# Azure/mmlspark

Hardware: NVIDIA H100
Metric: boosting_iters_per_sec (higher is better)
Workload: dtype int64 fixed-point histograms over u8 bins (fp32 gradients, fp64 split gains)

## Files before the change

mmlspark_b200/csrc/hist_kernel.cuh:

```cuda
#pragma once
#include <cstdint>
#include <cuda_runtime.h>
#include <cub/block/block_scan.cuh>

namespace b200gbm {

constexpr int kTileFeat = 32;
constexpr int kBins = 256;
constexpr int kLoBits = 18;
constexpr int kFlushRows = 1 << (32 - kLoBits);
#ifndef B200GBM_K4_EXPERIMENT
#define B200GBM_K4_EXPERIMENT 0
#endif
constexpr int kPlaneWords = kBins * kTileFeat;

struct HistWork {
  int begin;
  int count;
  int use_idx;
  int buf;
};

__global__ void __launch_bounds__(256)
k_gather_q(const HistWork* __restrict__ work, const int* __restrict__ idx0, const int* __restrict__ idx1, const int4* __restrict__ qgh,
           int4* __restrict__ qord) {
  const HistWork w = *work;
  if (!w.use_idx) return;
  const int* __restrict__ idx = w.buf ? idx1 : idx0;
  for (int i = blockIdx.x * blockDim.x + threadIdx.x; i < w.count; i += gridDim.x * blockDim.x) {
    const int p = w.begin + i;
    qord[p] = qgh[idx[p]];
  }
}

constexpr int kBoundBlockRows = 4096;
struct RowBlockBound {
  const int* prefix;
  int blocks;
};
inline int bound_blocks(int num_data) { return (num_data + kBoundBlockRows - 1) / kBoundBlockRows; }

__global__ void __launch_bounds__(256)
k_block_maxcnt(const uint8_t* __restrict__ bins, size_t rows_stride, int num_data, int num_columns, int* __restrict__ prefix) {
  __shared__ unsigned cnt[kBins * kTileFeat];
  __shared__ unsigned wmax[8];
  const int tile = blockIdx.y, tid = threadIdx.x;
  for (int e = tid; e < kBins * kTileFeat; e += blockDim.x) cnt[e] = 0u;
  __syncthreads();
  const int r0 = blockIdx.x * kBoundBlockRows, rows = min(kBoundBlockRows, num_data - r0);
  const unsigned* wp = reinterpret_cast<const unsigned*>(bins + (static_cast<size_t>(tile) * rows_stride + r0) * kTileFeat);
  for (int e = tid; e < rows * 8; e += blockDim.x) {
    const unsigned word = wp[e];
    const int c0 = (e & 7) * 4, rot = (e >> 3) & 3;
#pragma unroll
    for (int k = 0; k < 4; ++k) {
      const int kk = (k + rot) & 3;
      atomicAdd(&cnt[((word >> (8 * kk)) & 0xFFu) * kTileFeat + c0 + kk], 1u);
    }
  }
  __syncthreads();
  const int ncol = min(kTileFeat, num_columns - tile * kTileFeat);
  unsigned m = 0u;
  for (int e = tid; e < kBins * kTileFeat; e += blockDim.x)
    if ((e & (kTileFeat - 1)) < ncol) m = max(m, cnt[e]);
  m = __reduce_max_sync(0xffffffffu, m);
  if ((tid & 31) == 0) wmax[tid >> 5] = m;
  __syncthreads();
  if (tid == 0) {
    for (int i = 1; i < static_cast<int>(blockDim.x >> 5); ++i) m = max(m, wmax[i]);
    prefix[static_cast<size_t>(tile) * (gridDim.x + 1) + blockIdx.x] = static_cast<int>(m);
  }
}

__global__ void __launch_bounds__(1024) k_block_bound_prefix(int blocks, int* __restrict__ prefix) {
  using Scan = cub::BlockScan<int, 1024>;
  __shared__ typename Scan::TempStorage tmp;
  int* p = prefix + static_cast<size_t>(blockIdx.x) * (blocks + 1);
  int carry = 0;
  for (int b0 = 0; b0 < blocks; b0 += 1024) {
    const int b = b0 + threadIdx.x;
    const int v = b < blocks ? p[b] : 0;
    int ex, total;
    Scan(tmp).ExclusiveSum(v, ex, total);
    if (b < blocks) p[b] = carry + ex;
    carry += total;
    __syncthreads();
  }
  if (threadIdx.x == 0) p[blocks] = carry;
}

inline void launch_block_bound(const uint8_t* bins, size_t rows_stride, int num_data, int num_tiles, int num_columns, int* prefix,
                               cudaStream_t stream) {
  const int blocks = bound_blocks(num_data);
  if (blocks > 0) k_block_maxcnt<<<dim3(blocks, num_tiles), 256, 0, stream>>>(bins, rows_stride, num_data, num_columns, prefix);
  k_block_bound_prefix<<<num_tiles, 1024, 0, stream>>>(blocks, prefix);
}


__device__ __forceinline__ void cp_async16(void* smem, const void* gmem, bool valid) {
  unsigned s = static_cast<unsigned>(__cvta_generic_to_shared(smem));
  int sz = valid ? 16 : 0;
  asm volatile("cp.async.cg.shared.global [%0], [%1], 16, %2;\n" ::"r"(s), "l"(gmem), "r"(sz));
}
template <int N>
__device__ __forceinline__ void cp_async_wait() {
  asm volatile("cp.async.wait_group %0;\n" ::"n"(N));
}

constexpr int kWsConsumerWarps = 16;
constexpr int kWsProducerWarps = 2;
constexpr int kWsThreads = (kWsConsumerWarps + kWsProducerWarps) * 32;
constexpr int kWsStageRows = 512;
constexpr int kWsStages = 3;
constexpr int kFlushSlabBins = 32;
constexpr int kFlushRowBytes = kFlushSlabBins * 16;
constexpr int kFlushStageBytes = kTileFeat * kFlushRowBytes;
constexpr int kWsSmemBytes = 4 * kPlaneWords * 4 + kWsStages * (kWsStageRows * 32 + kWsStageRows * 16) + kFlushStageBytes + 64;
static_assert(kWsSmemBytes <= 227 * 1024, "K4 shared memory exceeds the 227 KB per block of sm_90");
static_assert(kFlushSlabBins * kTileFeat == 2 * kWsConsumerWarps * 32, "a flush slab is two (g,h) pairs per consumer thread");

__device__ __forceinline__ unsigned smem_u32(const void* p) { return static_cast<unsigned>(__cvta_generic_to_shared(p)); }
__device__ __forceinline__ void mbar_init(unsigned long long* bar, unsigned count) {
  asm volatile("mbarrier.init.shared::cta.b64 [%0], %1;\n" ::"r"(smem_u32(bar)), "r"(count));
}
__device__ __forceinline__ void mbar_arrive(unsigned long long* bar) {
  asm volatile("mbarrier.arrive.shared::cta.b64 _, [%0];\n" ::"r"(smem_u32(bar)) : "memory");
}
__device__ __forceinline__ void mbar_arrive_expect_tx(unsigned long long* bar, unsigned bytes) {
  asm volatile("mbarrier.arrive.expect_tx.shared::cta.b64 _, [%0], %1;\n" ::"r"(smem_u32(bar)), "r"(bytes) : "memory");
}
__device__ __forceinline__ void mbar_expect_tx(unsigned long long* bar, unsigned bytes) {
  asm volatile("mbarrier.expect_tx.relaxed.cta.shared::cta.b64 [%0], %1;\n" ::"r"(smem_u32(bar)), "r"(bytes) : "memory");
}
__device__ __forceinline__ void mbar_wait(unsigned long long* bar, unsigned parity) {
  asm volatile(
      "{\n"
      ".reg .pred p;\n"
      "WAIT_LOOP:\n"
      "mbarrier.try_wait.parity.shared::cta.b64 p, [%0], %1;\n"
      "@p bra DONE;\n"
      "bra WAIT_LOOP;\n"
      "DONE:\n"
      "}\n" ::"r"(smem_u32(bar)), "r"(parity) : "memory");
}
__device__ __forceinline__ void tma_bulk_g2s(void* smem_dst, const void* gmem_src, unsigned bytes, unsigned long long* bar) {
  asm volatile("cp.async.bulk.shared::cluster.global.mbarrier::complete_tx::bytes [%0], [%1], %2, [%3];\n" ::"r"(smem_u32(smem_dst)),
               "l"(gmem_src), "r"(bytes), "r"(smem_u32(bar))
               : "memory");
}
__device__ __forceinline__ void cp_async_mbar_arrive_noinc(unsigned long long* bar) {
  asm volatile("cp.async.mbarrier.arrive.noinc.shared::cta.b64 [%0];\n" ::"r"(smem_u32(bar)) : "memory");
}
__device__ __forceinline__ void bulk_reduce_add_u64(unsigned long long* gmem_dst, const void* smem_src, unsigned bytes) {
  asm volatile("cp.reduce.async.bulk.global.shared::cta.bulk_group.add.u64 [%0], [%1], %2;\n" ::"l"(gmem_dst), "r"(smem_u32(smem_src)),
               "r"(bytes)
               : "memory");
}
__device__ __forceinline__ void bulk_commit() { asm volatile("cp.async.bulk.commit_group;\n" ::: "memory"); }
__device__ __forceinline__ void bulk_wait_read_all() { asm volatile("cp.async.bulk.wait_group.read 0;\n" ::: "memory"); }
__device__ __forceinline__ void bulk_wait_all() { asm volatile("cp.async.bulk.wait_group 0;\n" ::: "memory"); }
__device__ __forceinline__ void fence_proxy_async_smem() { asm volatile("fence.proxy.async.shared::cta;\n" ::: "memory"); }

template <int NATOM>
__global__ void __launch_bounds__(kWsThreads, 1)
k4_hist_build_ws(const uint8_t* __restrict__ bins, size_t rows_stride, int num_tiles, const int4* __restrict__ qgh,
                 const int4* __restrict__ qord, const int* __restrict__ idx0, const int* __restrict__ idx1,
                 const HistWork* __restrict__ work, unsigned long long* __restrict__ hist, RowBlockBound bound) {
  extern __shared__ __align__(128) unsigned char smem_raw[];
  unsigned* plane = reinterpret_cast<unsigned*>(smem_raw);
  unsigned char* stage_bins = smem_raw + 4 * kPlaneWords * 4;
  int4* stage_q = reinterpret_cast<int4*>(stage_bins + kWsStages * kWsStageRows * 32);
  unsigned char* flush_stage = reinterpret_cast<unsigned char*>(stage_q) + kWsStages * kWsStageRows * 16;
  unsigned long long* full_bar = reinterpret_cast<unsigned long long*>(flush_stage + kFlushStageBytes);
  unsigned long long* empty_bar = full_bar + kWsStages;

  const HistWork w = *work;
  const int n = w.count;
  if (n <= 0) return;
  const int tid = threadIdx.x, lane = tid & 31, warp = tid >> 5;
  const int* __restrict__ idx = w.buf ? idx1 : idx0;

  long long cells_rows = static_cast<long long>(n) * num_tiles;
  int rpi = static_cast<int>((cells_rows + 4LL * gridDim.x - 1) / (4LL * gridDim.x));
  rpi = (rpi + kWsStageRows - 1) / kWsStageRows * kWsStageRows;
  rpi = max(rpi, kWsStageRows);
  rpi = min(rpi, kFlushRows);
  const int chunks = (n + rpi - 1) / rpi;
  const long long items = static_cast<long long>(chunks) * num_tiles;
  const int i0 = static_cast<int>(items * blockIdx.x / gridDim.x);
  const int i1 = static_cast<int>(items * (blockIdx.x + 1) / gridDim.x);
  if (i0 >= i1) return;

  if (tid == 0) {
    for (int i = 0; i < kWsStages; ++i) { mbar_init(&full_bar[i], kWsProducerWarps * 32); mbar_init(&empty_bar[i], kWsConsumerWarps); }
    asm volatile("fence.mbarrier_init.release.cluster;\n" ::: "memory");
  }
  for (int e = tid; e < 4 * kPlaneWords; e += kWsThreads) plane[e] = 0u;
  __syncthreads();

  unsigned gs = 0;
  if (warp >= kWsConsumerWarps) {
    const int ptid = tid - kWsConsumerWarps * 32;
    constexpr int kPT = kWsProducerWarps * 32;
    constexpr int kPerLane = kWsStageRows / kPT;
    for (int item = i0; item < i1; ++item) {
      const int tile = item / chunks, chunk = item - tile * chunks;
      const int row0 = chunk * rpi;
      const int nrows = min(rpi, n - row0);
      const int nst = (nrows + kWsStageRows - 1) / kWsStageRows;
      const uint8_t* tbins = bins + static_cast<size_t>(tile) * rows_stride * 32;
      for (int s = 0; s < nst; ++s, ++gs) {
        const int slot = gs % kWsStages;
        mbar_wait(&empty_bar[slot], ((gs / kWsStages) & 1u) ^ 1u);
        const int p0 = row0 + s * kWsStageRows;
        const int rows = min(kWsStageRows, row0 + nrows - p0);
        unsigned char* db = stage_bins + slot * kWsStageRows * 32;
        int4* dq = stage_q + slot * kWsStageRows;
        if (!w.use_idx) {
          if (ptid == 0) {
            mbar_arrive_expect_tx(&full_bar[slot], static_cast<unsigned>(rows) * 48u);
            const size_t r = static_cast<size_t>(w.begin + p0);
            tma_bulk_g2s(db, tbins + r * 32, static_cast<unsigned>(rows) * 32u, &full_bar[slot]);
            tma_bulk_g2s(dq, qgh + r, static_cast<unsigned>(rows) * 16u, &full_bar[slot]);
          } else {
            mbar_arrive(&full_bar[slot]);
          }
        } else {
          const int* ip = idx + w.begin + p0;
          if (ptid == 0) {
            mbar_expect_tx(&full_bar[slot], static_cast<unsigned>(rows) * 16u);
            tma_bulk_g2s(dq, qord + static_cast<size_t>(w.begin + p0), static_cast<unsigned>(rows) * 16u, &full_bar[slot]);
          }
          int rr[2 * kPerLane];
#pragma unroll
          for (int k = 0; k < 2 * kPerLane; ++k) { const int j = (ptid + k * kPT) >> 1; rr[k] = j < rows ? ip[j] : -1; }
#pragma unroll
          for (int k = 0; k < 2 * kPerLane; ++k) {
            const int hh = ptid + k * kPT, j = hh >> 1, half = (hh & 1) * 16;
            if (rr[k] >= 0) cp_async16(db + j * 32 + half, tbins + static_cast<size_t>(rr[k]) * 32 + half, true);
          }
          cp_async_mbar_arrive_noinc(&full_bar[slot]);
        }
      }
    }
    cp_async_wait<0>();
  } else {
#if B200GBM_K4_EXPERIMENT >= 1 && B200GBM_K4_EXPERIMENT <= 3
    unsigned exp_sink = 0;
#endif
    const int sub = lane >> 2, rot = lane & 3;
    auto item_rows = [&](int it, int& first, int& last) {
      const int t = it / chunks, r0 = (it - t * chunks) * rpi;
      first = w.begin + r0;
      last = first + min(rpi, n - r0) - 1;
      if (w.use_idx && bound.prefix) { first = idx[first]; last = idx[last]; }
    };
    auto item_bound = [&](int it, int first, int last) -> int {
      const int t = it / chunks, nr = min(rpi, n - (it - t * chunks) * rpi);
      if (!bound.prefix) return nr;
      const int* p = bound.prefix + static_cast<size_t>(t) * (bound.blocks + 1);
      return min(nr, p[last / kBoundBlockRows + 1] - p[first / kBoundBlockRows]);
    };
    int first, last;
    item_rows(i0, first, last);
    int next_bound = item_bound(i0, first, last);
    if (i0 + 1 < i1) item_rows(i0 + 1, first, last);
    int acc_bound = 0;
    for (int item = i0; item < i1; ++item) {
      const int tile = item / chunks, chunk = item - tile * chunks;
      const int row0 = chunk * rpi;
      const int nrows = min(rpi, n - row0);
      const int nst = (nrows + kWsStageRows - 1) / kWsStageRows;
      acc_bound += next_bound;
      next_bound = 0;
      if (item + 1 < i1) {
        next_bound = item_bound(item + 1, first, last);
        if (item + 2 < i1) item_rows(item + 2, first, last);
      }
      for (int s = 0; s < nst; ++s, ++gs) {
        const int slot = gs % kWsStages;
        mbar_wait(&full_bar[slot], (gs / kWsStages) & 1u);
        const int rows = min(kWsStageRows, nrows - s * kWsStageRows);
        const unsigned* sw = reinterpret_cast<const unsigned*>(stage_bins + slot * kWsStageRows * 32);
        const int4* sq = stage_q + slot * kWsStageRows;
        const int groups = (rows + 31) >> 5;
        for (int g = warp; g < groups; g += kWsConsumerWarps) {
          const int r = g * 32 + lane;
          if (r < rows) {
            const int4 q = sq[r];
            const unsigned* rw = sw + r * 8;
#pragma unroll
            for (int k = 0; k < 8; ++k) {
              const int w8 = (sub + k) & 7;
              const unsigned word = rw[w8];
#pragma unroll
              for (int j = 0; j < 4; ++j) {
                const int kk = (j + rot) & 3;
                const unsigned b = (word >> (8 * kk)) & 0xFFu;
                const unsigned a = b * 32u + static_cast<unsigned>(w8 * 4 + kk);
#if B200GBM_K4_EXPERIMENT == 0 || B200GBM_K4_EXPERIMENT == 4
                atomicAdd(&plane[a], static_cast<unsigned>(q.x));
                atomicAdd(&plane[kPlaneWords + a], static_cast<unsigned>(q.y));
                atomicAdd(&plane[2 * kPlaneWords + a], static_cast<unsigned>(q.z));
                if (NATOM == 4) atomicAdd(&plane[3 * kPlaneWords + a], static_cast<unsigned>(q.w));
#else
                if (B200GBM_K4_EXPERIMENT >= 2) atomicAdd(&plane[a], static_cast<unsigned>(q.x));
                if (B200GBM_K4_EXPERIMENT >= 3) atomicAdd(&plane[kPlaneWords + a], static_cast<unsigned>(q.y));
                if (B200GBM_K4_EXPERIMENT == 1) exp_sink ^= a + static_cast<unsigned>(q.x ^ q.y ^ q.z ^ q.w);
#endif
              }
            }
          }
        }
#if B200GBM_K4_EXPERIMENT >= 1 && B200GBM_K4_EXPERIMENT <= 3
        if (exp_sink == 0x12345679u) plane[lane] = exp_sink;
#endif
        __syncwarp();
        if (lane == 0) mbar_arrive(&empty_bar[slot]);
      }
      const bool flush = (item + 1 == i1) || ((item + 1) / chunks != tile) || (acc_bound + next_bound > kFlushRows);
      if (!flush) continue;
      acc_bound = 0;
      asm volatile("bar.sync 1, %0;\n" ::"n"(kWsConsumerWarps * 32) : "memory");
      unsigned long long* htile = hist + static_cast<size_t>(tile) * kTileFeat * kBins * 2;
      int sbin[2];
#pragma unroll
      for (int i = 0; i < 2; ++i) sbin[i] = (warp + i * kWsConsumerWarps + lane) & (kFlushSlabBins - 1);
      for (int b0 = 0; b0 < kBins; b0 += kFlushSlabBins) {
        long long g[2], h[2];
        bool nz = false;
#pragma unroll
        for (int i = 0; i < 2; ++i) {
          const int e = (b0 + sbin[i]) * kTileFeat + lane;
          const unsigned ghi = plane[e], glo = plane[kPlaneWords + e], hhi = plane[2 * kPlaneWords + e];
          const unsigned hlo = (NATOM == 4) ? plane[3 * kPlaneWords + e] : 0u;
          plane[e] = 0u;
          plane[kPlaneWords + e] = 0u;
          plane[2 * kPlaneWords + e] = 0u;
          if (NATOM == 4) plane[3 * kPlaneWords + e] = 0u;
          nz |= (ghi | glo | hhi | hlo) != 0u;
          g[i] = (static_cast<long long>(static_cast<int>(ghi)) << kLoBits) + static_cast<long long>(glo);
          h[i] = (NATOM == 4) ? (static_cast<long long>(static_cast<int>(hhi)) << kLoBits) + static_cast<long long>(hlo)
                              : static_cast<long long>(hhi);
        }
        if (tid == 0) bulk_wait_read_all();
        asm volatile("bar.sync 1, %0;\n" ::"n"(kWsConsumerWarps * 32) : "memory");
#pragma unroll
        for (int i = 0; i < 2; ++i)
          *reinterpret_cast<longlong2*>(flush_stage + lane * kFlushRowBytes + sbin[i] * 16) = make_longlong2(g[i], h[i]);
        fence_proxy_async_smem();
        int any;
        asm volatile(
            "{\n"
            ".reg .pred p, q;\n"
            "setp.ne.u32 p, %1, 0;\n"
            "bar.red.or.pred q, 1, %2, p;\n"
            "selp.s32 %0, 1, 0, q;\n"
            "}\n"
            : "=r"(any)
            : "r"(static_cast<unsigned>(nz)), "n"(kWsConsumerWarps * 32)
            : "memory");
#if B200GBM_K4_EXPERIMENT != 4
        if (tid == 0 && any) {
          for (int f = 0; f < kTileFeat; ++f)
            bulk_reduce_add_u64(htile + (static_cast<size_t>(f) * kBins + b0) * 2, flush_stage + f * kFlushRowBytes, kFlushSlabBins * 16);
          bulk_commit();
        }
#else
        (void)any; (void)htile;
#endif
      }
    }
    if (tid == 0) bulk_wait_all();
  }
}

inline cudaError_t set_k4_smem_limit() {
  const cudaError_t e = cudaFuncSetAttribute(k4_hist_build_ws<4>, cudaFuncAttributeMaxDynamicSharedMemorySize, kWsSmemBytes);
  if (e != cudaSuccess) return e;
  return cudaFuncSetAttribute(k4_hist_build_ws<3>, cudaFuncAttributeMaxDynamicSharedMemorySize, kWsSmemBytes);
}

inline void launch_k4(bool const_hessian, const uint8_t* bins, size_t rows_stride, int num_tiles, const int4* qgh, const int4* qord,
                      const int* idx0, const int* idx1, const HistWork* work, unsigned long long* hist, RowBlockBound bound, int grid,
                      cudaStream_t stream) {
  if (const_hessian)
    k4_hist_build_ws<3><<<grid, kWsThreads, kWsSmemBytes, stream>>>(bins, rows_stride, num_tiles, qgh, qord, idx0, idx1, work, hist, bound);
  else
    k4_hist_build_ws<4><<<grid, kWsThreads, kWsSmemBytes, stream>>>(bins, rows_stride, num_tiles, qgh, qord, idx0, idx1, work, hist, bound);
}

}
```

mmlspark_b200/csrc/tree_learner.cu:

```cuda
#include "tree_learner.h"

namespace b200gbm {

static size_t Align16(size_t x) { return (x + 15) & ~static_cast<size_t>(15); }
constexpr int kScanSmem = (768 + 64) * 8;
constexpr int kPartTickets = 8;

template <typename Fn>
static void ForEachTreeField(TreeDev& t, int L, Fn fn) {
  const size_t nodes = L - 1, leaves = L;
  fn(t.left_child, nodes); fn(t.right_child, nodes); fn(t.split_feature_inner, nodes); fn(t.threshold_bin, nodes);
  fn(t.decision_type, nodes); fn(t.split_gain, nodes); fn(t.leaf_value, leaves); fn(t.leaf_weight, leaves); fn(t.leaf_count, leaves);
  fn(t.internal_value, nodes); fn(t.internal_weight, nodes); fn(t.internal_count, nodes); fn(t.leaf_parent, leaves);
  fn(t.leaf_depth, leaves); fn(t.num_leaves, 1); fn(t.cat_bits, 8 * nodes); fn(t.cat_list, kCatListMax * nodes); fn(t.cat_list_len, nodes);
}
static size_t TreeBlobBytes(int L) {
  TreeDev t{};
  size_t bytes = 0;
  ForEachTreeField(t, L, [&](auto*& p, size_t count) { bytes += Align16(count * sizeof(*p)); });
  return bytes;
}
static TreeDev TreeBlobAt(unsigned char* base, int L) {
  TreeDev t{};
  size_t off = 0;
  ForEachTreeField(t, L, [&](auto*& p, size_t count) {
    p = reinterpret_cast<std::remove_reference_t<decltype(p)>>(base + off);
    off += Align16(count * sizeof(*p));
  });
  return t;
}

TreeLearner::TreeLearner(const Dataset& train, const Config& cfg, const Objective& obj, bool parallel, bool same_device, int num_sms,
                         cudaStream_t stream, Booster::Timing& timing)
    : train_(train), cfg_(cfg), parallel_(parallel), same_device_(same_device), num_sms_(num_sms), stream_(stream), timing_(timing) {
  const int n = train.num_data;
  const int L = cfg.num_leaves;
  cudaDeviceSetLimit(cudaLimitMaxL2FetchGranularity, 32);
  cudaGetLastError();
  B200_CUDA(set_k4_smem_limit());
  B200_CUDA(cudaFuncSetAttribute(k_scan, cudaFuncAttributeMaxDynamicSharedMemorySize, kScanSmem));

  ResetConfig(cfg);
  sp_.num_leaves = L; sp_.parallel = parallel_ ? 1 : 0;
  sp_.nf = train.nf; sp_.nf_pad = train.nf_pad; sp_.num_tiles = train.num_tiles; sp_.nfn = train.nfn;
  {
    sp_.cat_l2 = cfg.cat_l2; sp_.cat_smooth = cfg.cat_smooth;
    sp_.max_cat_threshold = cfg.max_cat_threshold; sp_.max_cat_to_onehot = cfg.max_cat_to_onehot;
    sp_.min_data_per_group = cfg.min_data_per_group; sp_.pad3 = 0;
    if (train.nw > 0) {
      if (sp_.max_cat_threshold > kCatListMax) Fatal("max_cat_threshold > " + std::to_string(kCatListMax) + " is not supported together with categorical features of more than 256 bins");
      if (sp_.max_cat_to_onehot > 256) Fatal("max_cat_to_onehot > 256 is not supported together with categorical features of more than 256 bins");
      B200_CUDA(cudaFuncSetAttribute(k4_hist_wide<4>, cudaFuncAttributeMaxDynamicSharedMemorySize, 4 * kWideHistSeg * 4));
      B200_CUDA(cudaFuncSetAttribute(k4_hist_wide<3>, cudaFuncAttributeMaxDynamicSharedMemorySize, 4 * kWideHistSeg * 4));
      B200_CUDA(cudaFuncSetAttribute(k_scan_wide, cudaFuncAttributeMaxDynamicSharedMemorySize, kWideMaxBins * 8));
    }
  }

  qgh_.Alloc(n); qord_.Alloc(n); idx0_.Alloc(n); idx1_.Alloc(n);
  slot_elems_ = train.hist_pairs * 2;
  H_.Alloc(slot_elems_); H_.Zero(stream_); pool_.Alloc(slot_elems_ * L);
  {
    int per_sm = 0;
    B200_CUDA(cudaOccupancyMaxActiveBlocksPerMultiprocessor(&per_sm, k_partition, 256, 0));
    int coop = 0;
    cudaDeviceGetAttribute(&coop, cudaDevAttrCooperativeLaunch, CurrentDevice());
    if (!coop || per_sm < 1) Fatal("this device cannot launch the cooperative partition kernel");
    part_max_blocks_ = per_sm * num_sms_;
  }
  flags_.Alloc(static_cast<size_t>(L) * train.nf_pad);
  cands_.Alloc(2 * static_cast<size_t>(train.nf_pad));
  leaves_.Alloc(L); ctrl_.Alloc(1); ctrl_.Zero(stream_);
  const int chunks = n / kPartChunk + 2;
  part_bits_.Alloc(static_cast<size_t>(chunks) * (kPartChunk / 32)); part_chunks_.Alloc(static_cast<size_t>(chunks) + chunks / kPartLocalScan + 8); part_chunks_.Zero(stream_);
  const size_t blob_bytes = TreeBlobBytes(L);
  tree_blob_.Alloc(blob_bytes);
  tree_dev_ = TreeAt(tree_blob_.p);
  B200_CUDA(cudaMemsetAsync(tree_blob_.p, 0, blob_bytes, stream_));
  B200_CUDA(cudaMallocHost(reinterpret_cast<void**>(&tree_host_), blob_bytes));
  B200_CUDA(cudaMallocHost(reinterpret_cast<void**>(&ctrl_host_), sizeof(TreeCtrl)));
  if (obj.RenewsLeaves()) {
    rn_keys_a_.Alloc(n); rn_keys_b_.Alloc(n); rn_pos_a_.Alloc(n); rn_pos_b_.Alloc(n); rn_leaf_of_pos_.Alloc(n); rn_leaf_a_.Alloc(n); rn_leaf_b_.Alloc(n);
    rn_res_.Alloc(n); rn_row_.Alloc(n); rn_seg_.Alloc(L + 1); rn_out_.Alloc(2 * static_cast<size_t>(L));
    if (obj.RenewWeights()) rn_cdf_.Alloc(n);
    size_t t1 = 0, t2 = 0;
    cub::DeviceRadixSort::SortPairs(nullptr, t1, rn_keys_a_.p, rn_keys_b_.p, rn_pos_a_.p, rn_pos_b_.p, n, 0, 64, stream_);
    cub::DeviceRadixSort::SortPairs(nullptr, t2, rn_leaf_a_.p, rn_leaf_b_.p, rn_pos_b_.p, rn_pos_a_.p, n, 0, 32, stream_);
    rn_tmp_bytes_ = std::max(t1, t2);
    rn_tmp_.Alloc(rn_tmp_bytes_ + 16);
  }
  col_rand_ = LcgRandom(cfg.feature_fraction_seed);
  feature_used_host_.assign(train.nf_pad, 0);
  for (int u = 0; u < train.nf; ++u) feature_used_host_[u] = 1;
  feature_used_.Alloc(train.nf_pad);
  feature_used_.Upload(feature_used_host_.data(), train.nf_pad, stream_);
  ResetFeaturesByTree();
}

TreeLearner::~TreeLearner() {
  if (split_op_trees_ > 0) {
    double tot = 0; for (auto& kv : split_op_ms_) tot += kv.second;
    fprintf(stderr, "[b200gbm split timing] %d trees, %.3f ms per tree in split operations:", split_op_trees_, tot / split_op_trees_);
    for (auto& kv : split_op_ms_) fprintf(stderr, " %s=%.1fus", kv.first.c_str(), 1000.0 * kv.second / split_op_trees_ / std::max(cfg_.num_leaves - 1, 1));
    fprintf(stderr, " (per split)\n");
  }
  if (tree_host_) cudaFreeHost(tree_host_);
  if (ctrl_host_) cudaFreeHost(ctrl_host_);
}

void TreeLearner::ResetConfig(const Config& cfg) {
  sp_.l1 = cfg.lambda_l1; sp_.l2 = cfg.lambda_l2; sp_.max_delta_step = cfg.max_delta_step; sp_.min_gain_to_split = cfg.min_gain_to_split;
  sp_.min_sum_hessian = cfg.min_sum_hessian_in_leaf; sp_.min_data_in_leaf = cfg.min_data_in_leaf; sp_.max_depth = cfg.max_depth;
}

TreeDev TreeLearner::TreeAt(unsigned char* blob) const { return TreeBlobAt(blob, sp_.num_leaves); }

void TreeLearner::ResetFeaturesByTree() {
  if (cfg_.feature_fraction >= 1.0) return;
  const int total = train_.nf;
  int cnt = std::max(static_cast<int>(total * cfg_.feature_fraction + 0.5), std::min(2, total));
  std::fill(feature_used_host_.begin(), feature_used_host_.end(), 0);
  for (int i : col_rand_.Sample(total, cnt)) feature_used_host_[train_.sample_order[i]] = 1;
  feature_used_.Upload(feature_used_host_.data(), train_.nf_pad, stream_);
}

void TreeLearner::Renew(const Objective& obj, const double* score_k, double rf_pred) {
  const int total = rows_;
  const int L = cfg_.num_leaves;
  cudaStream_t s = stream_;
  TreeCtrl* ctrl = ctrl_.p;
  const int egrid = num_sms_ * 8;
  const float* wptr = obj.RenewWeights();
  k_renew_gather<<<egrid, 256, 0, s>>>(ctrl, leaves_.p, idx0_.p, idx1_.p, train_.d_label.p, score_k, rf_pred,
                                       rn_keys_a_.p, rn_pos_a_.p, rn_res_.p, rn_leaf_of_pos_.p, rn_row_.p);
  size_t tb = rn_tmp_bytes_;
  B200_CUDA(cub::DeviceRadixSort::SortPairs(rn_tmp_.p, tb, rn_keys_a_.p, rn_keys_b_.p, rn_pos_a_.p, rn_pos_b_.p, total, 0, 64, s));
  k_renew_leaf_keys<<<egrid, 256, 0, s>>>(rn_pos_b_.p, rn_leaf_of_pos_.p, total, rn_leaf_a_.p);
  int leaf_bits = 1;
  while ((1 << leaf_bits) < L) ++leaf_bits;
  tb = rn_tmp_bytes_;
  B200_CUDA(cub::DeviceRadixSort::SortPairs(rn_tmp_.p, tb, rn_leaf_a_.p, rn_leaf_b_.p, rn_pos_b_.p, rn_pos_a_.p, total, 0, leaf_bits, s));
  k_renew_offsets<<<1, 32, 0, s>>>(ctrl, leaves_.p, rn_seg_.p);
  double* out = rn_out_.p;
  double* has = rn_out_.p + L;
  const int lgrid = (L + 127) / 128;
  if (!wptr) {
    k_renew_unweighted<<<lgrid, 128, 0, s>>>(ctrl, rn_seg_.p, rn_pos_a_.p, rn_res_.p, obj.RenewAlpha(), out, has);
  } else {
    k_renew_cdf<<<L, 1024, 0, s>>>(ctrl, rn_seg_.p, rn_pos_a_.p, rn_row_.p, wptr, rn_cdf_.p);
    k_renew_weighted<<<lgrid, 128, 0, s>>>(ctrl, rn_seg_.p, rn_pos_a_.p, rn_res_.p, rn_cdf_.p, obj.RenewAlpha(), out, has);
  }
  if (parallel_) Net().AllReduce(out, 2 * static_cast<size_t>(L), ncclDouble, ncclSum, s);
  k_renew_apply<<<lgrid, 128, 0, s>>>(ctrl, tree_dev_, out, has, parallel_ ? 1 : 0);
  B200_CUDA(cudaGetLastError());
  timing_.launches += wptr ? 7 : 6;
}

void TreeLearner::EnsureColumnCopy() {
  if (cols_tried_) return;
  cols_tried_ = true;
  const Dataset& d = train_;
  const char* env = std::getenv("B200GBM_COLUMN_COPY");
  if ((env && std::atoi(env) == 0) || d.nfn == 0) return;
  size_t free_b = 0, total_b = 0;
  const bool mem_ok = cudaMemGetInfo(&free_b, &total_b) == cudaSuccess;
  if (!mem_ok) cudaGetLastError();
  size_t share = 1;
  if (same_device_) {
    double arrived = 0.0;
    AllReduceHost(&arrived, 1, ncclSum, stream_);
    if (cudaMemGetInfo(&free_b, &total_b) != cudaSuccess) { cudaGetLastError(); free_b = 0; }
    double f = mem_ok ? static_cast<double>(free_b) : 0.0;
    AllReduceHost(&f, 1, ncclMin, stream_);
    free_b = static_cast<size_t>(f);
    share = static_cast<size_t>(Net().world);
  }
  if (!mem_ok || d.num_data == 0) return;
  const char* force = std::getenv("B200GBM_COLUMN_CACHE_COLUMNS");
  const size_t stride = (static_cast<size_t>(d.num_data) + 255) & ~static_cast<size_t>(255);
  const int ncols = d.num_tiles * 32;
  const size_t need = static_cast<size_t>(ncols) * stride;
  const size_t reserve = std::max<size_t>(static_cast<size_t>(8) << 30, total_b / 10);
  const size_t spare = free_b > reserve ? (free_b - reserve) / share : 0;
  const bool full = !force && spare >= need;
  int slots = ncols;
  if (!full) {
    slots = static_cast<int>(std::min<size_t>(d.num_columns, spare / stride));
    if (force) slots = std::min(slots, std::max(0, std::atoi(force)));
    if (slots == 0) return;
  }
  const size_t bytes = static_cast<size_t>(slots) * stride;
  uint8_t* p = nullptr;
  if (cudaMalloc(reinterpret_cast<void**>(&p), bytes) != cudaSuccess) { cudaGetLastError(); return; }
  bins_cols_.p = p; bins_cols_.n = bytes;
  cols_stride_ = stride;
  col_slot_host_.assign(ncols, -1);
  if (full) {
    for (int c = 0; c < ncols; ++c) col_slot_host_[c] = c;
    const long long work = ((static_cast<long long>(d.num_data) + 255) / 256) * d.num_tiles;
    k_tiles_to_columns<<<static_cast<unsigned>(std::min<long long>(work, static_cast<long long>(num_sms_) * 16)), 256, 0, stream_>>>(
        d.bins.p, d.rows_stride, d.num_tiles, d.num_data, bins_cols_.p, stride);
    B200_CUDA(cudaGetLastError());
  } else {
    slot_col_.assign(slots, -1);
    col_splits_.assign(ncols, 0);
  }
  col_slot_.Alloc(ncols);
  col_slot_.Upload(col_slot_host_.data(), ncols, stream_);
}

void TreeLearner::UpdateColumnCache(const HostTree& t) {
  if (slot_col_.empty()) return;
  const Dataset& d = train_;
  for (int i = 0; i + 1 < t.num_leaves; ++i) {
    const int f = t.split_feature_inner[i];
    if (f < d.nfn) ++col_splits_[d.meta_host[f].hist_off >> 8];
  }
  std::vector<int> cand;
  for (int c = 0; c < static_cast<int>(col_splits_.size()); ++c)
    if (col_splits_[c] > 0 && col_slot_host_[c] < 0) cand.push_back(c);
  std::stable_sort(cand.begin(), cand.end(), [&](int a, int b) { return col_splits_[a] > col_splits_[b]; });
  ColumnJobs jobs{};
  for (int c : cand) {
    if (jobs.n == kColumnBuildsMax) break;
    int slot = -1, victim = -1;
    for (int s = 0; s < static_cast<int>(slot_col_.size()) && slot < 0; ++s) {
      const int held = slot_col_[s];
      if (held < 0) slot = s;
      else if (victim < 0 || col_splits_[held] < col_splits_[slot_col_[victim]]) victim = s;
    }
    if (slot < 0) {
      if (col_splits_[slot_col_[victim]] >= col_splits_[c]) break;
      slot = victim;
      col_slot_host_[slot_col_[slot]] = -1;
      ++cache_evictions_;
    }
    slot_col_[slot] = c;
    col_slot_host_[c] = slot;
    jobs.col[jobs.n] = c; jobs.slot[jobs.n] = slot; ++jobs.n;
  }
  if (jobs.n == 0) return;
  const long long words = (static_cast<long long>(d.num_data) + 3) / 4;
  const unsigned gx = static_cast<unsigned>(std::max<long long>(1, std::min<long long>((words + 255) / 256, static_cast<long long>(num_sms_) * 8)));
  k_tiles_to_column_slots<<<dim3(gx, jobs.n), 256, 0, stream_>>>(d.bins.p, d.rows_stride, d.num_data, jobs, bins_cols_.p, cols_stride_);
  B200_CUDA(cudaGetLastError());
  col_slot_.Upload(col_slot_host_.data(), col_slot_host_.size(), stream_);
  cache_builds_ += jobs.n;
  timing_.launches += 1;
}

void TreeLearner::GetColumnCacheInfo(int64_t* out4) const {
  out4[0] = static_cast<int64_t>(slot_col_.size());
  out4[1] = static_cast<int64_t>(std::count_if(slot_col_.begin(), slot_col_.end(), [](int c) { return c >= 0; }));
  out4[2] = cache_builds_;
  out4[3] = cache_evictions_;
}

void TreeLearner::LaunchPartition(int grid, int last) {
  const Dataset& d = train_;
  TreeCtrl* ctrl = ctrl_.p;
  LeafState* leaves = leaves_.p;
  TreeDev tree = tree_dev_;
  uint8_t* flags = flags_.p;
  const FeatMeta* meta = d.meta.p;
  SplitParams sp = sp_;
  const uint8_t* bins = d.bins.p;
  size_t rows_stride = d.rows_stride;
  int* i0 = idx0_.p; int* i1 = idx1_.p;
  unsigned* bits = part_bits_.p;
  int* chunks = part_chunks_.p;
  const int4* qgh = qgh_.p;
  int4* qord = qord_.p;
  long long* H = H_.p;
  size_t h_elems = slot_elems_;
  const uint16_t* bins16 = d.bins16.p;
  int tickets_per_block = kPartTickets;
  const uint8_t* cols = bins_cols_.p;
  size_t cols_stride = cols_stride_;
  const int* col_slot = col_slot_.p;
  int* super_tot = part_chunks_.p + (d.num_data / kPartChunk + 2);
  const int* bundle_base = d.BundleBase();
  void* args[] = {&ctrl, &leaves, &tree, &flags, &meta, &sp, &last, &bins, &rows_stride, &i0, &i1, &bits, &chunks, &qgh, &qord, &H, &h_elems, &bins16, &tickets_per_block,
                  &cols, &cols_stride, &col_slot, &super_tot, &bundle_base};
  B200_CUDA(cudaLaunchCooperativeKernel(reinterpret_cast<void*>(k_partition), dim3(grid), dim3(256), args, 0, stream_));
}

void TreeLearner::Grow(const float* g, const float* h, bool const_hessian, const Bag* bag) {
  EnsureColumnCopy();
  const Dataset& d = train_;
  const int n = d.num_data;
  const int L = cfg_.num_leaves;
  rows_ = bag ? bag->count : n;
  TreeCtrl* ctrl = ctrl_.p;
  cudaStream_t s = stream_;
  const int egrid = num_sms_ * 8;
  nvtxRangePushA("b200gbm:K3 quantize + C1 root sums");
  B200_CUDA(cudaMemsetAsync(&ctrl->absmax_bits[0], 0, 8, s));
  k_absmax<<<egrid, 256, 0, s>>>(g, h, n, ctrl);
  if (parallel_) Net().AllReduce(&ctrl->absmax_bits[0], 2, ncclUint32, ncclMax, s);
  k_set_scale<<<1, 1, 0, s>>>(ctrl, const_hessian ? 1 : 0, 1.0);
  k_quantize<<<egrid, 256, 0, s>>>(g, h, n, qgh_.p, ctrl, const_hessian ? 1 : 0, bag ? bag->in_bag : nullptr, rows_);
  if (parallel_) Net().AllReduce(&ctrl->root_q[0], 3, ncclInt64, ncclSum, s);
  ResetFeaturesByTree();
  if (bag)
    B200_CUDA(cudaMemcpyAsync(idx0_.p, bag->rows, static_cast<size_t>(bag->count) * sizeof(int), cudaMemcpyDeviceToDevice, s));
  k_tree_init<<<1, 256, 0, s>>>(ctrl, leaves_.p, tree_dev_, flags_.p, sp_, rows_, feature_used_.p, bag ? 1 : 0);
  nvtxRangePop();
  timing_.launches += 4;
  const int pgrid = std::max(1, std::min(n / kPartChunk + 1, part_max_blocks_));
  const dim3 sgrid(std::max(1, d.nfn), 2);
  const RowBlockBound bound = d.BlockBound();
  static const bool split_timing = getenv("B200GBM_SPLIT_TIMING") != nullptr;
  auto mark = [&]() { if (split_timing) { cudaEvent_t e; cudaEventCreate(&e); cudaEventRecord(e, s); split_events_.push_back(e); } };
  k_round_ctl<<<1, 256, 0, s>>>(ctrl, leaves_.p, tree_dev_, flags_.p, d.meta.p, sp_, 0);
  timing_.launches += 1;
  for (int split = 0; split < L - 1; ++split) {
    mark();
    if (profile_hist) { cudaEvent_t a, b; B200_CUDA(cudaEventCreate(&a)); B200_CUDA(cudaEventCreate(&b)); hist_events_.push_back(a); hist_events_.push_back(b); B200_CUDA(cudaEventRecord(a, s)); }
    if (split == 0 && bag) k_gather_q<<<egrid, 256, 0, s>>>(&ctrl->hist_work, idx0_.p, idx1_.p, qgh_.p, qord_.p);
    mark();
    nvtxRangePushA("b200gbm:K4 histogram");
    launch_k4(const_hessian, d.bins.p, d.rows_stride, d.num_tiles, qgh_.p, qord_.p, idx0_.p, idx1_.p, &ctrl->hist_work,
              reinterpret_cast<unsigned long long*>(H_.p), bound, num_sms_, s);
    if (d.nw > 0) {
      int max_nb = 0;
      for (const WideMeta& wm : d.wide_host) max_nb = std::max(max_nb, wm.num_bin);
      const int segs = (max_nb + kWideHistSeg - 1) / kWideHistSeg;
      int units = 0;
      for (const WideMeta& wm : d.wide_host) units += (wm.num_bin + kWideHistSeg - 1) / kWideHistSeg;
      const dim3 wgrid(static_cast<unsigned>(std::max(1, std::min(64, 4 * num_sms_ / std::max(1, units)))), static_cast<unsigned>(d.nw), static_cast<unsigned>(segs));
      if (const_hessian)
        k4_hist_wide<3><<<wgrid, kWideThreads, 4 * kWideHistSeg * 4, s>>>(d.bins16.p, d.rows_stride, d.wide_meta.p, qgh_.p, qord_.p, idx0_.p, idx1_.p, &ctrl->hist_work,
                                                                         reinterpret_cast<unsigned long long*>(H_.p));
      else
        k4_hist_wide<4><<<wgrid, kWideThreads, 4 * kWideHistSeg * 4, s>>>(d.bins16.p, d.rows_stride, d.wide_meta.p, qgh_.p, qord_.p, idx0_.p, idx1_.p, &ctrl->hist_work,
                                                                         reinterpret_cast<unsigned long long*>(H_.p));
      timing_.launches += 1;
    }
    nvtxRangePop();
    if (profile_hist) B200_CUDA(cudaEventRecord(hist_events_.back(), s));
    mark();
    nvtxRangePushA(parallel_ ? "b200gbm:C2 histogram reduce + K5 scan + pick" : "b200gbm:K5 scan + pick");
    if (parallel_) Net().AllReduce(H_.p, slot_elems_, ncclInt64, ncclSum, s);
    mark();
    if (d.nw > 0) {
      k_scan_wide<<<dim3(d.nw, 2), 256, kWideMaxBins * 8, s>>>(ctrl, leaves_.p, d.wide_meta.p, H_.p, pool_.p, slot_elems_, flags_.p, cands_.p, sp_);
      timing_.launches += 1;
    }
    k_scan<<<sgrid, 256, (d.has_categorical || !d.bundles.empty()) ? kScanSmem : 0, s>>>(ctrl, leaves_.p, d.meta.p, H_.p, pool_.p, slot_elems_, flags_.p, cands_.p, sp_, d.BundleBase());
    nvtxRangePop();
    mark();
    nvtxRangePushA("b200gbm:K7 partition + controller");
    LaunchPartition(pgrid, split == L - 2 ? 1 : 0);
    nvtxRangePop();
    mark();
    timing_.launches += 3; timing_.hist_launches += 1;
  }
}

void TreeLearner::AddScore(double* score_k, double shrinkage) {
  k_add_score<<<num_sms_ * 8, 256, 0, stream_>>>(ctrl_.p, leaves_.p, tree_dev_, idx0_.p, idx1_.p, score_k, shrinkage);
}

void TreeLearner::ReadTree(HostTree* out) {
  const Dataset& d = train_;
  cudaStream_t s = stream_;
  B200_CUDA(cudaMemcpyAsync(tree_host_, tree_blob_.p, tree_blob_.n, cudaMemcpyDeviceToHost, s));
  B200_CUDA(cudaMemcpyAsync(ctrl_host_, ctrl_.p, sizeof(TreeCtrl), cudaMemcpyDeviceToHost, s));
  B200_CUDA(cudaStreamSynchronize(s));
  if (!split_events_.empty()) {
    static const char* kOps[] = {"gather_q(bagged root)", "K4", "allreduce", "scan+pick", "partition+zeroH+ctl"};
    const int per = 6;
    for (size_t b0 = 0; b0 + per <= split_events_.size(); b0 += per)
      for (int o = 0; o < per - 1; ++o) { float ms = 0; cudaEventElapsedTime(&ms, split_events_[b0 + o], split_events_[b0 + o + 1]); split_op_ms_[kOps[o]] += ms; }
    split_op_trees_ += 1;
    for (auto e : split_events_) cudaEventDestroy(e);
    split_events_.clear();
  }
  if (!hist_events_.empty()) {
    for (size_t i = 0; i + 1 < hist_events_.size(); i += 2) { float ms = 0; cudaEventElapsedTime(&ms, hist_events_[i], hist_events_[i + 1]); timing_.hist_ms += ms; }
    for (auto e : hist_events_) cudaEventDestroy(e);
    hist_events_.clear();
  }
  timing_.hist_rows += ctrl_host_->trace_rows;
  const TreeDev t = TreeAt(tree_host_);
  const int nl = *t.num_leaves;
  out->Resize(nl);
  if (nl > 1) {
    for (int i = 0; i < nl - 1; ++i) {
      const int sf = t.split_feature_inner[i], tb = t.threshold_bin[i], dt = t.decision_type[i];
      out->left_child[i] = t.left_child[i]; out->right_child[i] = t.right_child[i]; out->split_feature_inner[i] = sf;
      out->split_feature[i] = d.used[sf]; out->threshold_in_bin[i] = static_cast<uint32_t>(tb);
      out->decision_type[i] = static_cast<int8_t>(dt); out->split_gain[i] = t.split_gain[i];
      const FeatureBins& fbm = d.mappers[d.used[sf]];
      if (dt & 1) {
        std::vector<int> cats;
        if (sf >= d.nfn) { for (int k = 0; k < t.cat_list_len[i]; ++k) cats.push_back(fbm.bin_to_cat[t.cat_list[i * kCatListMax + k]]); }
        else for (int b = 0; b < fbm.num_bin; ++b) if ((t.cat_bits[i * 8 + (b >> 5)] >> (b & 31)) & 1u) cats.push_back(fbm.bin_to_cat[b]);
        out->AddCategoricalNode(i, cats);
      } else {
        double thr = fbm.upper[tb];
        if (std::isnan(thr)) thr = 0.0; else if (thr >= 1e300) thr = 1e300; else if (thr <= -1e300) thr = -1e300;
        out->threshold[i] = thr;
      }
      out->internal_value[i] = t.internal_value[i]; out->internal_weight[i] = t.internal_weight[i]; out->internal_count[i] = t.internal_count[i];
    }
    for (int i = 0; i < nl; ++i) { out->leaf_value[i] = t.leaf_value[i]; out->leaf_weight[i] = t.leaf_weight[i]; out->leaf_count[i] = t.leaf_count[i]; out->leaf_depth[i] = t.leaf_depth[i]; }
  } else {
    out->leaf_value[0] = 0.0;
  }
  UpdateColumnCache(*out);
}

}
```

mmlspark_b200/csrc/tree_learner.h:

```cpp
#pragma once
#include "engine.h"

namespace b200gbm {

class TreeLearner {
 public:
  TreeLearner(const Dataset& train, const Config& cfg, const Objective& obj, bool parallel, bool same_device, int num_sms,
              cudaStream_t stream, Booster::Timing& timing);
  ~TreeLearner();
  void ResetConfig(const Config& cfg);

  struct Bag { const uint8_t* in_bag; const int* rows; int count; };
  void Grow(const float* g, const float* h, bool const_hessian, const Bag* bag);
  void Renew(const Objective& obj, const double* score_k, double rf_pred);
  void AddScore(double* score_k, double shrinkage);
  const TreeDev& Tree() const { return tree_dev_; }
  const DevBuf<unsigned char>& Blob() const { return tree_blob_; }
  TreeDev TreeAt(unsigned char* blob) const;
  void ReadTree(HostTree* out);

  bool profile_hist = false;
  size_t ColumnCopyBytes() const { return bins_cols_.n; }
  void GetColumnCacheInfo(int64_t* out4) const;

 private:
  void ResetFeaturesByTree();
  void LaunchPartition(int grid, int last);
  void EnsureColumnCopy();
  void UpdateColumnCache(const HostTree& t);

  const Dataset& train_;
  const Config& cfg_;
  const bool parallel_, same_device_;
  const int num_sms_;
  cudaStream_t stream_;
  Booster::Timing& timing_;
  SplitParams sp_{};
  int rows_ = 0;
  DevBuf<int4> qgh_, qord_;
  DevBuf<int> idx0_, idx1_;
  DevBuf<long long> H_;
  DevBuf<long long> pool_;
  size_t slot_elems_ = 0;
  DevBuf<uint8_t> flags_;
  DevBuf<SplitCand> cands_;
  DevBuf<LeafState> leaves_;
  DevBuf<TreeCtrl> ctrl_;
  DevBuf<unsigned char> tree_blob_;
  TreeDev tree_dev_{};
  unsigned char* tree_host_ = nullptr;
  TreeCtrl* ctrl_host_ = nullptr;
  DevBuf<unsigned> part_bits_;
  DevBuf<int> part_chunks_;
  int part_max_blocks_ = 0;
  DevBuf<uint8_t> bins_cols_;
  size_t cols_stride_ = 0;
  bool cols_tried_ = false;
  DevBuf<int> col_slot_;
  std::vector<int> col_slot_host_;
  std::vector<int> slot_col_;
  std::vector<long long> col_splits_;
  long long cache_builds_ = 0, cache_evictions_ = 0;
  LcgRandom col_rand_{2};
  std::vector<uint8_t> feature_used_host_;
  DevBuf<uint8_t> feature_used_;
  DevBuf<unsigned long long> rn_keys_a_, rn_keys_b_;
  DevBuf<unsigned> rn_pos_a_, rn_pos_b_, rn_leaf_of_pos_, rn_leaf_a_, rn_leaf_b_;
  DevBuf<double> rn_res_, rn_cdf_, rn_out_;
  DevBuf<int> rn_row_, rn_seg_;
  DevBuf<unsigned char> rn_tmp_;
  size_t rn_tmp_bytes_ = 0;
  std::vector<cudaEvent_t> split_events_, hist_events_;
  std::map<std::string, double> split_op_ms_;
  int split_op_trees_ = 0;
};

}
```

Baseline: 6.490.

## Assign histogram work items to CTAs aligned per tile with strided chunks

Changes how the warp-specialized histogram kernel splits (tile, chunk) items across CTAs. When the grid is a multiple of the tile count and rows are indexed, each CTA stays on one tile and takes strided chunks, and leftover chunks are spread over the remaining CTAs. The goal is to avoid CTAs whose item range crosses tiles, which forces extra shared-to-global flushes and causes imbalance. Per-split profiling also gains a separate timing for the root K4 launch. The flush condition now relies on the next item's tile, which changes when partial histograms are flushed.

After: 6.675 (median of 6 runs). 2.8% higher.

```diff
diff --git a/mmlspark_b200/csrc/hist_kernel.cuh b/mmlspark_b200/csrc/hist_kernel.cuh
--- a/mmlspark_b200/csrc/hist_kernel.cuh
+++ b/mmlspark_b200/csrc/hist_kernel.cuh
@@ -165,7 +165,7 @@
 __global__ void __launch_bounds__(kWsThreads, 1)
 k4_hist_build_ws(const uint8_t* __restrict__ bins, size_t rows_stride, int num_tiles, const int4* __restrict__ qgh,
                  const int4* __restrict__ qord, const int* __restrict__ idx0, const int* __restrict__ idx1,
-                 const HistWork* __restrict__ work, unsigned long long* __restrict__ hist, RowBlockBound bound) {
+                 const HistWork* __restrict__ work, unsigned long long* __restrict__ hist, RowBlockBound bound, bool aligned) {
   extern __shared__ __align__(128) unsigned char smem_raw[];
   unsigned* plane = reinterpret_cast<unsigned*>(smem_raw);
   unsigned char* stage_bins = smem_raw + 4 * kPlaneWords * 4;
@@ -186,10 +186,30 @@
   rpi = max(rpi, kWsStageRows);
   rpi = min(rpi, kFlushRows);
   const int chunks = (n + rpi - 1) / rpi;
-  const long long items = static_cast<long long>(chunks) * num_tiles;
-  const int i0 = static_cast<int>(items * blockIdx.x / gridDim.x);
-  const int i1 = static_cast<int>(items * (blockIdx.x + 1) / gridDim.x);
-  if (i0 >= i1) return;
+  const int R = (aligned && w.use_idx) ? static_cast<int>(gridDim.x) / num_tiles : 0;
+  const int per_cta = static_cast<int>((static_cast<long long>(chunks) * num_tiles + gridDim.x - 1) / gridDim.x);
+  const int creg = min(chunks, per_cta * R), ctail = chunks - creg;
+  const bool regular = static_cast<int>(blockIdx.x) < R * num_tiles;
+  int i0 = 0, nitems;
+  if (regular) {
+    const int j = blockIdx.x % R;
+    nitems = j < creg ? (creg - 1 - j) / R + 1 : 0;
+  } else {
+    const int e = blockIdx.x - R * num_tiles, ne = gridDim.x - R * num_tiles;
+    const long long items = static_cast<long long>(ctail) * num_tiles;
+    i0 = static_cast<int>(items * e / ne);
+    nitems = static_cast<int>(items * (e + 1) / ne) - i0;
+  }
+  if (nitems <= 0) return;
+  auto item_at = [&](int k, int& tile, int& chunk) {
+    if (regular) {
+      tile = blockIdx.x / R;
+      chunk = blockIdx.x % R + k * R;
+    } else {
+      tile = (i0 + k) / ctail;
+      chunk = creg + i0 + k - tile * ctail;
+    }
+  };
 
   if (tid == 0) {
     for (int i = 0; i < kWsStages; ++i) { mbar_init(&full_bar[i], kWsProducerWarps * 32); mbar_init(&empty_bar[i], kWsConsumerWarps); }
@@ -203,8 +223,9 @@
     const int ptid = tid - kWsConsumerWarps * 32;
     constexpr int kPT = kWsProducerWarps * 32;
     constexpr int kPerLane = kWsStageRows / kPT;
-    for (int item = i0; item < i1; ++item) {
-      const int tile = item / chunks, chunk = item - tile * chunks;
+    for (int it = 0; it < nitems; ++it) {
+      int tile, chunk;
+      item_at(it, tile, chunk);
       const int row0 = chunk * rpi;
       const int nrows = min(rpi, n - row0);
       const int nst = (nrows + kWsStageRows - 1) / kWsStageRows;
@@ -249,33 +270,39 @@
     unsigned exp_sink = 0;
 #endif
     const int sub = lane >> 2, rot = lane & 3;
-    auto item_rows = [&](int it, int& first, int& last) {
-      const int t = it / chunks, r0 = (it - t * chunks) * rpi;
+    auto item_rows = [&](int k, int& first, int& last) {
+      int t, c;
+      item_at(k, t, c);
+      const int r0 = c * rpi;
       first = w.begin + r0;
       last = first + min(rpi, n - r0) - 1;
       if (w.use_idx && bound.prefix) { first = idx[first]; last = idx[last]; }
     };
-    auto item_bound = [&](int it, int first, int last) -> int {
-      const int t = it / chunks, nr = min(rpi, n - (it - t * chunks) * rpi);
+    auto item_bound = [&](int k, int first, int last) -> int {
+      int t, c;
+      item_at(k, t, c);
+      const int nr = min(rpi, n - c * rpi);
       if (!bound.prefix) return nr;
       const int* p = bound.prefix + static_cast<size_t>(t) * (bound.blocks + 1);
       return min(nr, p[last / kBoundBlockRows + 1] - p[first / kBoundBlockRows]);
     };
     int first, last;
-    item_rows(i0, first, last);
-    int next_bound = item_bound(i0, first, last);
-    if (i0 + 1 < i1) item_rows(i0 + 1, first, last);
+    item_rows(0, first, last);
+    int next_bound = item_bound(0, first, last);
+    if (1 < nitems) item_rows(1, first, last);
     int acc_bound = 0;
-    for (int item = i0; item < i1; ++item) {
-      const int tile = item / chunks, chunk = item - tile * chunks;
+    for (int it = 0; it < nitems; ++it) {
+      int tile, chunk, next_tile = -1, next_chunk;
+      item_at(it, tile, chunk);
+      if (it + 1 < nitems) item_at(it + 1, next_tile, next_chunk);
       const int row0 = chunk * rpi;
       const int nrows = min(rpi, n - row0);
       const int nst = (nrows + kWsStageRows - 1) / kWsStageRows;
       acc_bound += next_bound;
       next_bound = 0;
-      if (item + 1 < i1) {
-        next_bound = item_bound(item + 1, first, last);
-        if (item + 2 < i1) item_rows(item + 2, first, last);
+      if (it + 1 < nitems) {
+        next_bound = item_bound(it + 1, first, last);
+        if (it + 2 < nitems) item_rows(it + 2, first, last);
       }
       for (int s = 0; s < nst; ++s, ++gs) {
         const int slot = gs % kWsStages;
@@ -318,7 +345,7 @@
         __syncwarp();
         if (lane == 0) mbar_arrive(&empty_bar[slot]);
       }
-      const bool flush = (item + 1 == i1) || ((item + 1) / chunks != tile) || (acc_bound + next_bound > kFlushRows);
+      const bool flush = (next_tile != tile) || (acc_bound + next_bound > kFlushRows);
       if (!flush) continue;
       acc_bound = 0;
       asm volatile("bar.sync 1, %0;\n" ::"n"(kWsConsumerWarps * 32) : "memory");
@@ -383,11 +410,18 @@
 
 inline void launch_k4(bool const_hessian, const uint8_t* bins, size_t rows_stride, int num_tiles, const int4* qgh, const int4* qord,
                       const int* idx0, const int* idx1, const HistWork* work, unsigned long long* hist, RowBlockBound bound, int grid,
+                      bool aligned, cudaStream_t stream) {
+  if (const_hessian)
+    k4_hist_build_ws<3><<<grid, kWsThreads, kWsSmemBytes, stream>>>(bins, rows_stride, num_tiles, qgh, qord, idx0, idx1, work, hist, bound,
+                                                                    aligned);
+  else
+    k4_hist_build_ws<4><<<grid, kWsThreads, kWsSmemBytes, stream>>>(bins, rows_stride, num_tiles, qgh, qord, idx0, idx1, work, hist, bound,
+                                                                    aligned);
+}
+inline void launch_k4(bool const_hessian, const uint8_t* bins, size_t rows_stride, int num_tiles, const int4* qgh, const int4* qord,
+                      const int* idx0, const int* idx1, const HistWork* work, unsigned long long* hist, RowBlockBound bound, int num_sms,
                       cudaStream_t stream) {
-  if (const_hessian)
-    k4_hist_build_ws<3><<<grid, kWsThreads, kWsSmemBytes, stream>>>(bins, rows_stride, num_tiles, qgh, qord, idx0, idx1, work, hist, bound);
-  else
-    k4_hist_build_ws<4><<<grid, kWsThreads, kWsSmemBytes, stream>>>(bins, rows_stride, num_tiles, qgh, qord, idx0, idx1, work, hist, bound);
-}
-
-}
+  launch_k4(const_hessian, bins, rows_stride, num_tiles, qgh, qord, idx0, idx1, work, hist, bound, num_sms, true, stream);
+}
+
+}
diff --git a/mmlspark_b200/csrc/tree_learner.cu b/mmlspark_b200/csrc/tree_learner.cu
--- a/mmlspark_b200/csrc/tree_learner.cu
+++ b/mmlspark_b200/csrc/tree_learner.cu
@@ -101,7 +101,8 @@
     double tot = 0; for (auto& kv : split_op_ms_) tot += kv.second;
     fprintf(stderr, "[b200gbm split timing] %d trees, %.3f ms per tree in split operations:", split_op_trees_, tot / split_op_trees_);
     for (auto& kv : split_op_ms_) fprintf(stderr, " %s=%.1fus", kv.first.c_str(), 1000.0 * kv.second / split_op_trees_ / std::max(cfg_.num_leaves - 1, 1));
-    fprintf(stderr, " (per split)\n");
+    fprintf(stderr, " (per split); K4 split 0=%.1fus, K4 splits 1+=%.1fus\n", 1000.0 * split_k4_root_ms_ / split_op_trees_,
+            1000.0 * (split_op_ms_["K4"] - split_k4_root_ms_) / split_op_trees_ / std::max(cfg_.num_leaves - 2, 1));
   }
   if (tree_host_) cudaFreeHost(tree_host_);
   if (ctrl_host_) cudaFreeHost(ctrl_host_);
@@ -371,7 +372,12 @@
     static const char* kOps[] = {"gather_q(bagged root)", "K4", "allreduce", "scan+pick", "partition+zeroH+ctl"};
     const int per = 6;
     for (size_t b0 = 0; b0 + per <= split_events_.size(); b0 += per)
-      for (int o = 0; o < per - 1; ++o) { float ms = 0; cudaEventElapsedTime(&ms, split_events_[b0 + o], split_events_[b0 + o + 1]); split_op_ms_[kOps[o]] += ms; }
+      for (int o = 0; o < per - 1; ++o) {
+        float ms = 0;
+        cudaEventElapsedTime(&ms, split_events_[b0 + o], split_events_[b0 + o + 1]);
+        split_op_ms_[kOps[o]] += ms;
+        if (b0 == 0 && o == 1) split_k4_root_ms_ += ms;
+      }
     split_op_trees_ += 1;
     for (auto e : split_events_) cudaEventDestroy(e);
     split_events_.clear();
diff --git a/mmlspark_b200/csrc/tree_learner.h b/mmlspark_b200/csrc/tree_learner.h
--- a/mmlspark_b200/csrc/tree_learner.h
+++ b/mmlspark_b200/csrc/tree_learner.h
@@ -73,6 +73,7 @@
   std::vector<cudaEvent_t> split_events_, hist_events_;
   std::map<std::string, double> split_op_ms_;
   int split_op_trees_ = 0;
+  double split_k4_root_ms_ = 0;
 };
 
 }
```
